# TheNeodev/RVC-MAKER

Hardware: AMD Instinct MI355X
Metric: audio-seconds/sec/GPU (xRT) end-to-end VC, 48k v2; 1/2/4/8 GPU scaling (higher is better)
Workload: dtype f32-equivalent (split-fp16 3-pass MFMA for the generator's convs -- scale from the producer's published |max| -- and ResBlock pairs, split-bf16 6-pass MFMA elsewhere; f32 accumulate; RMVPE f64 with its GRU recurrence f32); 1 GPU; VC.pipeline 48k v2, ContentVec-768, rmvpe f0, one 30 s clip per GPU per step, no index, protect 0.33, clip stream (clip k+1 f0/features under clip k synthesizer); model=RVC v2 48k (NSF-HiFiGAN) + ContentVec + rmvpe, global_batch=1, seq_len=480000, parallelism=utterance-sharded x1

## Files before the change

include/rvc_amd.h:

```cpp
#ifndef RVC_AMD_H
#define RVC_AMD_H

#include <stdint.h>

#ifdef __cplusplus
extern "C" {
#endif

typedef struct ihipStream_t* rvc_stream_t;

enum { RVC_OK = 0, RVC_EINVAL = -22, RVC_EHIP = -5 };

enum {
    RVC_ACT_NONE = 0,
    RVC_ACT_LRELU = 1,
    RVC_ACT_RELU = 2,
    RVC_ACT_TANH = 3,
    RVC_ACT_GELU = 4,
    RVC_ACT_SIGMOID = 5,
    RVC_ACT_LOGCLAMP = 6,
};

const char* rvc_last_error(void);
int rvc_version(void);
// ... 19 lines not shown
    int ntoff, wrap;
    int toff[16];
    const void* wx;
    int wx_nmf, wx_passes;
    const unsigned* amax_in;
    unsigned* amax_out;
    const float* src_x;
    const float* src_w;
    const float* src_b;
    int src_K, src_stride, src_pad, _pad1;
    int64_t src_len, src_bstride;
} rvc_conv1d_args;

int64_t rvc_conv1d_workspace_bytes(const rvc_conv1d_args* a);
int rvc_conv1d_engine(const rvc_conv1d_args* a);
int rvc_conv1d(const rvc_conv1d_args* a, void* ws, int64_t ws_bytes, rvc_stream_t stream);
void rvc_conv1d_set_probe_event(void* hip_event);
int rvc_conv1d_set_stamps(void* buf, int64_t bytes);
int rvc_resblock_set_stamps(void* buf, int64_t bytes);
int rvc_resblock_set_ylds(int on);
int rvc_resblock_set_wide64(int on);
int rvc_conv1d_set_tile_epi(int on);
int rvc_conv1d_set_swz(int on);
int rvc_conv1d_set_f16_fast(int on);
int rvc_conv1d_set_splitk_target(int target);
int rvc_stream_create_cu_mask(const uint32_t* mask, int nwords, rvc_stream_t* out);
int rvc_stream_destroy(rvc_stream_t stream);
int64_t rvc_conv1d_x6_bytes(int64_t nphase, int64_t Ci, int K, int64_t Co);
int rvc_conv1d_pack_x6(const float* w_km, int64_t nphase, int64_t Ci, int K, int64_t Co, void* out, int* nmf_out,
                       rvc_stream_t stream);
// ... 323 lines not shown
```

rvc-maker_amd/csrc/conv1d.hip:

```cpp
#include "rvc_common.h"
#include "x6_common.h"
#include <stdlib.h>
#include <type_traits>
#include <algorithm>

namespace {

constexpr int KCH = 32;
constexpr int NB_MAX = 16;

struct ConvParams {
    const float* x;
    const float* w;
    const float* bias;
    const float* bias2;
    const float* res;
    float* y;
    float* ws;
    int64_t B, Ci, Co, Lin, Lout, ncols;
    int64_t x_bstride, y_bstride, res_bstride, w_bstride;
    int K, stride, dil, pad, groups;
    int nphase, ostride, ooffset;
    int in_act, out_act, accumulate;
    float in_scale, in_slope, out_slope, out_scale;
// ... 51 lines not shown
    else if (t <= -2) yb[m * p.Lout + (-t - 2)] = 0.f;
    return ok ? v : 0.f;
}

template <int ACT, int FM, int FN>
__device__ __forceinline__ void apply_act(floatx4 (&acc)[FM][FN], float slope, float scale) {
#pragma unroll
    for (int i = 0; i < FM; ++i)
#pragma unroll
        for (int j = 0; j < FN; ++j)
#pragma unroll
            for (int r = 0; r < 4; ++r) acc[i][j][r] = act_apply(acc[i][j][r], ACT, slope) * scale;
}

template <int FM, int FN, int WM, int WN>
__device__ __forceinline__ void conv_epilogue(const ConvParams& p, floatx4 (&acc)[FM][FN], int lane, int wm, int wn,
                                              int split, int phase, int b, int g, int Cog, int m0g, int64_t n0) {
    const int ln = lane & 15;
    const int lr = (lane >> 4) * 4;
    if (p.ksplit > 1) {
        float* wsb = p.ws + (((int64_t)split * p.B * p.nphase + (int64_t)b * p.nphase + phase) * p.Co) * p.ncols;
#pragma unroll
        for (int i = 0; i < FM; ++i)
#pragma unroll
            for (int r = 0; r < 4; ++r) {
                const int mg = m0g + wm * 16 * FM + i * 16 + lr + r;
                const int64_t m = (int64_t)g * Cog + mg;
#pragma unroll
                for (int j = 0; j < FN; ++j) {
                    const int64_t n = n0 + wn * 16 * FN + j * 16 + ln;
                    if (mg < Cog && n < p.ncols) wsb[m * p.ncols + n] = acc[i][j][r];
                }
            }
        return;
    }
    int tcol[FN];
#pragma unroll
    for (int j = 0; j < FN; ++j) tcol[j] = out_pos(p, n0 + wn * 16 * FN + j * 16 + ln, phase);
    float* yb = p.y + b * p.y_bstride;
    const float* rb2 = p.res ? p.res + b * p.res_bstride : nullptr;
    const int Lo = (int)p.Lout;
    float amx = 0.f;
#pragma unroll
    for (int i = 0; i < FM; ++i) {
        floatx4 (&av)[1][FN] = *reinterpret_cast<floatx4 (*)[1][FN]>(&acc[i][0]);
        int mrow[4];
        bool mok[4];
#pragma unroll
        for (int r = 0; r < 4; ++r) {
            const int mg = m0g + wm * 16 * FM + i * 16 + lr + r;
            mok[r] = mg < Cog;
            mrow[r] = g * Cog + (mg < Cog ? mg : 0);
            float bs = 0.f;
            if (p.bias) bs = p.bias[mrow[r]];
            if (p.bias2) bs += p.bias2[mrow[r]];
#pragma unroll
            for (int j = 0; j < FN; ++j) av[0][j][r] += bs;
        }
        switch (p.out_act) {
            case RVC_ACT_LRELU: apply_act<RVC_ACT_LRELU, 1, FN>(av, p.out_slope, p.out_scale); break;
            case RVC_ACT_RELU: apply_act<RVC_ACT_RELU, 1, FN>(av, p.out_slope, p.out_scale); break;
            case RVC_ACT_TANH: apply_act<RVC_ACT_TANH, 1, FN>(av, p.out_slope, p.out_scale); break;
            case RVC_ACT_GELU: apply_act<RVC_ACT_GELU, 1, FN>(av, p.out_slope, p.out_scale); break;
            case RVC_ACT_SIGMOID: apply_act<RVC_ACT_SIGMOID, 1, FN>(av, p.out_slope, p.out_scale); break;
            case RVC_ACT_LOGCLAMP: apply_act<RVC_ACT_LOGCLAMP, 1, FN>(av, p.out_slope, p.out_scale); break;
            default: apply_act<RVC_ACT_NONE, 1, FN>(av, p.out_slope, p.out_scale); break;
        }
        if (rb2) {
#pragma unroll
            for (int r = 0; r < 4; ++r)
// ... 11 lines not shown
#pragma unroll
            for (int j = 0; j < FN; ++j) {
                if (mok[r] && tcol[j] >= 0) {
                    yb[mrow[r] * Lo + tcol[j]] = av[0][j][r];
                    amx = fmaxf(amx, fabsf(av[0][j][r]));
                } else if (mok[r] && tcol[j] <= -2) {
                    yb[mrow[r] * Lo + (-tcol[j] - 2)] = 0.f;
                }
            }
    }
    if (p.amax_out) amax_publish(p.amax_out + (int64_t)b * RVC_AMAX_SHARDS, amx);
}

template <int FM, int FN, int WM, int WN>
__device__ __forceinline__ void conv_epilogue_swz(const ConvParams& p, floatx4 (&acc)[FM][FN], int lane, int wm, int wn,
                                                  int phase, int b, int g, int Cog, int m0g, int64_t n0) {
    static_assert(FN % 2 == 0, "column fragments in pairs");
    constexpr int NP = FN / 2;
    const int h = lane >> 5, lc = lane & 31;
    int tcol[NP];
#pragma unroll
    for (int jp = 0; jp < NP; ++jp) tcol[jp] = out_pos(p, n0 + wn * 16 * FN + jp * 32 + lc, phase);
    float* yb = p.y + b * p.y_bstride;
    const float* rb2 = p.res ? p.res + b * p.res_bstride : nullptr;
    const int Lo = (int)p.Lout;
    float amx = 0.f;
#pragma unroll
    for (int i = 0; i < FM; ++i) {
#pragma unroll
        for (int jp = 0; jp < NP; ++jp)
#pragma unroll
            for (int r = 0; r < 4; ++r) {
                const auto sw = __builtin_amdgcn_permlane16_swap(__float_as_uint(acc[i][2 * jp][r]),
                                                                 __float_as_uint(acc[i][2 * jp + 1][r]), false, false);
                acc[i][2 * jp][r] = __uint_as_float(sw[0]);
                acc[i][2 * jp + 1][r] = __uint_as_float(sw[1]);
            }
        floatx4 (&av)[1][FN] = *reinterpret_cast<floatx4 (*)[1][FN]>(&acc[i][0]);
        int mrow[8];
        bool mok[8];
#pragma unroll
        for (int k = 0; k < 8; ++k) {
            const int mg = m0g + wm * 16 * FM + i * 16 + 8 * h + k;
            mok[k] = mg < Cog;
            mrow[k] = g * Cog + (mg < Cog ? mg : 0);
            float bs = 0.f;
            if (p.bias) bs = p.bias[mrow[k]];
            if (p.bias2) bs += p.bias2[mrow[k]];
#pragma unroll
            for (int jp = 0; jp < NP; ++jp) av[0][2 * jp + (k >> 2)][k & 3] += bs;
        }
        switch (p.out_act) {
            case RVC_ACT_LRELU: apply_act<RVC_ACT_LRELU, 1, FN>(av, p.out_slope, p.out_scale); break;
            case RVC_ACT_RELU: apply_act<RVC_ACT_RELU, 1, FN>(av, p.out_slope, p.out_scale); break;
            case RVC_ACT_TANH: apply_act<RVC_ACT_TANH, 1, FN>(av, p.out_slope, p.out_scale); break;
            case RVC_ACT_GELU: apply_act<RVC_ACT_GELU, 1, FN>(av, p.out_slope, p.out_scale); break;
            case RVC_ACT_SIGMOID: apply_act<RVC_ACT_SIGMOID, 1, FN>(av, p.out_slope, p.out_scale); break;
            case RVC_ACT_LOGCLAMP: apply_act<RVC_ACT_LOGCLAMP, 1, FN>(av, p.out_slope, p.out_scale); break;
            default: apply_act<RVC_ACT_NONE, 1, FN>(av, p.out_slope, p.out_scale); break;
        }
        if (rb2) {
#pragma unroll
            for (int k = 0; k < 8; ++k)
// ... 9 lines not shown
                    av[0][2 * jp + (k >> 2)][k & 3] += yb[mrow[k] * Lo + (tcol[jp] >= 0 ? tcol[jp] : 0)];
        }
#pragma unroll
        for (int k = 0; k < 8; ++k)
#pragma unroll
            for (int jp = 0; jp < NP; ++jp) {
                const float v = av[0][2 * jp + (k >> 2)][k & 3];
                if (mok[k] && tcol[jp] >= 0) {
                    yb[mrow[k] * Lo + tcol[jp]] = v;
                    amx = fmaxf(amx, fabsf(v));
                } else if (mok[k] && tcol[jp] <= -2) {
                    yb[mrow[k] * Lo + (-tcol[jp] - 2)] = 0.f;
                }
            }
    }
    if (p.amax_out) amax_publish(p.amax_out + (int64_t)b * RVC_AMAX_SHARDS, amx);
}

template <int FM, int FN, int WM, int WN>
__global__ __launch_bounds__(256) void conv1d_mfma_kernel(ConvParams p) {
    constexpr int BM = 16 * FM * WM;
    constexpr int BN = 16 * FN * WN;
    constexpr int WS = (BM / 32) * 32 + 16 + ((BM % 32) ? 32 : 0);
    constexpr int NA = KCH * BM / 256;
    constexpr bool AVEC_OK = (NA % 4) == 0 && (BM % 4) == 0;
    extern __shared__ __attribute__((aligned(16))) float smem[];
    float* Ws = smem;
    int* koff = (int*)(smem + KCH * WS);
    float* Xs = smem + KCH * WS + KCH;

// ... 285 lines not shown
    if (p.amax_out && !part) amax_publish(p.amax_out + (int64_t)b * RVC_AMAX_SHARDS, amx);
}

template <int FM, int FN, int WM, int WN, int X6_NI, int NP, bool F16, bool SA = false, int LF = 0>
__global__ __launch_bounds__(64 * (WM * WN + 4), (x6_min_blocks<FM, FN, WM * WN, NP>())) void conv_x6_kernel(ConvParams p) {
    static_assert(WM * WN == 4 || WM * WN == 8, "4 or 8 compute waves");
    constexpr int NCW = WM * WN;
    static_assert(NP == 6 || NP == 3 || NP == 1, "6, 3 or 1 passes");
    static_assert(!F16 || NP == 3, "split-fp16: 3 passes");
    static_assert(!SA || (NP == 6 && !F16), "split accumulators: 6-pass split-bf16");
    static_assert(LF == 0 || (F16 && WM * WN == 8), "fast-only loaders: split-fp16 on 8 compute waves");
    constexpr int NPL = NP == 6 ? 3 : (NP == 3 ? 2 : 1);
    constexpr int BM = 16 * FM * WM;
    constexpr int BN = 16 * FN * WN;
    extern __shared__ uint4 xs[];
    const int tid = threadIdx.x, lane = tid & 63, wave = tid >> 6;
    int bx = blockIdx.x, by = blockIdx.y, bz = blockIdx.z;
    if (p.xcd) {
        const int nx = gridDim.x, ny = gridDim.y;
        const int nwg = nx * ny * (int)gridDim.z;
        const int orig = bx + nx * (by + ny * bz);
        const int q = nwg >> 3, r = nwg & 7, xc = orig & 7;
        const int t = (xc < r ? xc * (q + 1) : r * (q + 1) + (xc - r) * q) + (orig >> 3);
        bx = t % nx;
        by = (t / nx) % ny;
        bz = t / (nx * ny);
    }
    int zb = bz;
    const int split = zb % p.ksplit;
    zb /= p.ksplit;
    const int phase = zb % p.nphase;
    const int b = zb / p.nphase;
    const int grp = p.gx6 ? phase : 0;
    const int ophase = p.gx6 ? 0 : phase;
    const int Cog = (int)p.Co;
    const int Cig = (int)p.Ci;
    const int m0g = by * BM;
    const int64_t n0 = (int64_t)bx * BN;
    const int K = p.K, span = p.span;
    const int nch = p.wx_nch, nmf = p.wx_nmf;
    const int ch_beg = split * p.chunks_per_split;
    const int ch_end = min(nch, ch_beg + p.chunks_per_split);
    const int nck = ch_end - ch_beg;
    const int bufsz = NPL * span * 4;
    float* tmax = reinterpret_cast<float*>(xs + 2 * bufsz);
    const int rseed = p.rot ? (bx >> 3) : 0;
    const int rt = rseed % K, rc = (rseed / K) % max(nck, 1);
    auto pchunk = [&](int i) __attribute__((always_inline)) {
        const int c = min(i, nck - 1) + rc;
        return ch_beg + (c >= nck ? c - nck : c);
    };

    if (p.stagger) {
        const int lin = blockIdx.x + gridDim.x * (blockIdx.y + gridDim.y * blockIdx.z);
        if (lin < p.stagger_blocks) {
            const unsigned long long t0 = X6_NOW();
            const unsigned long long d = ((unsigned long long)((lin * 97) & 255) * (unsigned)p.stagger) >> 8;
            while (X6_NOW() - t0 < d) __builtin_amdgcn_s_sleep(2);
        }
    }
// ... 213 lines not shown
                x6_tile_epilogue<BM / 2, BN, 64 * (NCW + 4)>(p, reinterpret_cast<const float*>(xs), tid, split, b, m0g,
                                                             n0);
                __syncthreads();
                __syncthreads();
                x6_tile_epilogue<BM / 2, BN, 64 * (NCW + 4)>(p, reinterpret_cast<const float*>(xs), tid, split, b,
                                                             m0g + BM / 2, n0);
            }
        }
        return;
    }

    const int wm = wave / WN, wn = wave % WN;
    const int s_beg = ch_beg * K, s_end = ch_end * K;
    const uint4* wxp = p.wx + (int64_t)phase * K * nch * nmf * 3 * 64;
    const int mf0 = m0g / 16 + wm * FM;
    auto aload = [&](int i, int tl, uint4 (&a)[NPL][FM]) __attribute__((always_inline)) {
        const int ch = pchunk(i);
        const int t = tl + rt < K ? tl + rt : tl + rt - K;
        const int frag0 = __builtin_amdgcn_readfirstlane((t * nch + ch) * nmf + mf0);
        const uint4* src = wxp + (int64_t)frag0 * 3 * 64;
#pragma unroll
        for (int i = 0; i < FM; ++i)
#pragma unroll
            for (int q = 0; q < NPL; ++q) a[q][i] = src[(i * 3 + q) * 64 + lane];
    };
    floatx4 acc[FM][FN];
    floatx4 acc_lo[SA ? FM : 1][SA ? FN : 1];
#pragma unroll
    for (int i = 0; i < FM; ++i)
#pragma unroll
// ... 53 lines not shown
    uint4 abuf[NB][NPL][FM];
    int li = 0, lt = 0;
#pragma unroll
    for (int i = 0; i < PD; ++i) {
        aload(li, lt, abuf[i]);
        if (++lt == K) { lt = 0; ++li; }
    }
    float tile_rs = 1.f;
    if (wave == 0) X6_STAMP(3, X6_NOW());
    if constexpr (F16) {
        if (!(LF || p.amax_in)) {
            __syncthreads();
            tile_rs = ldexpf(1.f, -f16_exp(fmaxf(fmaxf(tmax[0], tmax[1]), fmaxf(tmax[2], tmax[3]))));
        }
        if (wave == 0) X6_STAMP(4, X6_NOW());
    }
    __syncthreads();
    if constexpr (F16) {
        if (LF || p.amax_in) tile_rs = ldexpf(1.f, -f16_exp(fmaxf(fmaxf(tmax[0], tmax[1]), fmaxf(tmax[2], tmax[3]))));
    }
    if (wave == 0) X6_STAMP(5, X6_NOW());
    const int nsteps = s_end - s_beg;
    int ci = 0, ct = 0;
    for (int s0 = 0; s0 < nsteps; s0 += NB) {
#pragma unroll
        for (int u = 0; u < NB; ++u) {
            aload(li, lt, abuf[(u + PD) % NB]);
            if (++lt == K) { lt = 0; ++li; }
            __builtin_amdgcn_sched_barrier(0);
            if (s0 + u < nsteps) {
// ... 8 lines not shown
    }
    if (wave == 0) X6_STAMP(6, X6_NOW());
    if constexpr (SA) {
#pragma unroll
        for (int i = 0; i < FM; ++i)
#pragma unroll
            for (int j = 0; j < FN; ++j)
#pragma unroll
                for (int r = 0; r < 4; ++r) acc[i][j][r] += acc_lo[i][j][r];
    }
    if (kAblations && (p.dbg & 1)) {
        if (acc[0][0][0] == 1234.5f) p.y[lane] = acc[FM - 1][FN - 1][3];
        return;
    }
    if constexpr (F16) {
        const float* rs = reinterpret_cast<const float*>(p.wx + (int64_t)p.nphase * K * nch * nmf * 3 * 64);
#pragma unroll
        for (int i = 0; i < FM; ++i)
#pragma unroll
            for (int r = 0; r < 4; ++r) {
                const float f = rs[m0g + wm * 16 * FM + i * 16 + lg * 4 + r] * tile_rs;
#pragma unroll
                for (int j = 0; j < FN; ++j) acc[i][j][r] *= f;
            }
    }
    if (BN <= 128 && p.tile_epi) {
        float* ot = reinterpret_cast<float*>(xs);
        constexpr int TS = BN + 4;
#pragma unroll
        for (int i = 0; i < FM; ++i) {
            floatx4 (&av)[1][FN] = *reinterpret_cast<floatx4 (*)[1][FN]>(&acc[i][0]);
            if (p.ksplit == 1) {
#pragma unroll
                for (int r = 0; r < 4; ++r) {
                    const int mg = m0g + wm * 16 * FM + i * 16 + lg * 4 + r;
                    const int mr = mg < Cog ? mg : 0;
                    float bs = 0.f;
                    if (p.bias) bs = p.bias[mr];
                    if (p.bias2) bs += p.bias2[mr];
#pragma unroll
                    for (int j = 0; j < FN; ++j) av[0][j][r] += bs;
                }
                switch (p.out_act) {
                    case RVC_ACT_LRELU: apply_act<RVC_ACT_LRELU, 1, FN>(av, p.out_slope, p.out_scale); break;
                    case RVC_ACT_RELU: apply_act<RVC_ACT_RELU, 1, FN>(av, p.out_slope, p.out_scale); break;
                    case RVC_ACT_TANH: apply_act<RVC_ACT_TANH, 1, FN>(av, p.out_slope, p.out_scale); break;
                    case RVC_ACT_GELU: apply_act<RVC_ACT_GELU, 1, FN>(av, p.out_slope, p.out_scale); break;
                    case RVC_ACT_SIGMOID: apply_act<RVC_ACT_SIGMOID, 1, FN>(av, p.out_slope, p.out_scale); break;
                    case RVC_ACT_LOGCLAMP: apply_act<RVC_ACT_LOGCLAMP, 1, FN>(av, p.out_slope, p.out_scale); break;
                    default: apply_act<RVC_ACT_NONE, 1, FN>(av, p.out_slope, p.out_scale); break;
                }
            }
        }
        auto put = [&](int row0) __attribute__((always_inline)) {
// ... 6 lines not shown
                        ot[(wm * 16 * FM - row0 + i * 16 + lg * 4 + r) * TS + wn * 16 * FN + j * 16 + ln] = acc[i][j][r];
        };
        if (p.tile_epi == 1) {
            put(0);
            __syncthreads();
            x6_tile_epilogue<BM, BN, 64 * (NCW + 4)>(p, ot, tid, split, b, m0g, n0);
        } else if constexpr (WM % 2 == 0) {
            if (wm < WM / 2) put(0);
            __syncthreads();
            x6_tile_epilogue<BM / 2, BN, 64 * (NCW + 4)>(p, ot, tid, split, b, m0g, n0);
            __syncthreads();
            if (wm >= WM / 2) put(BM / 2);
            __syncthreads();
            x6_tile_epilogue<BM / 2, BN, 64 * (NCW + 4)>(p, ot, tid, split, b, m0g + BM / 2, n0);
        }
    } else if (p.swz && p.ksplit == 1) {
        conv_epilogue_swz<FM, FN, WM, WN>(p, acc, lane, wm, wn, ophase, b, grp, Cog, m0g, n0);
    } else {
        conv_epilogue<FM, FN, WM, WN>(p, acc, lane, wm, wn, split, ophase, b, grp, Cog, m0g, n0);
    }
#if RVC_CONV_STAMPS
    if (wave == 0) {
        X6_STAMP(14, X6_NOW());
        __builtin_amdgcn_s_waitcnt(0);
        X6_STAMP(7, X6_NOW());
    }
#endif
}

constexpr int RED_ROWS = 8;
__global__ __launch_bounds__(256) void conv_splitk_reduce(ConvParams p) {
    const int64_t n = (int64_t)blockIdx.x * blockDim.x + threadIdx.x;
    const int bp = blockIdx.z, b = bp / p.nphase;
    const int64_t m0 = (int64_t)blockIdx.y * RED_ROWS;
// ... 298 lines not shown
    }

    if (x6_eligible(a)) {
        cfg.x6 = true;
        static const int w8 = getenv("RVC_X6_W8") ? atoi(getenv("RVC_X6_W8")) : 1;
        const int np = a->wx_passes == 0 || a->wx_passes == RVC_ARITH_FP32_SA ? 6 : a->wx_passes;
        static const int bn256 = getenv("RVC_X6_BN256") ? atoi(getenv("RVC_X6_BN256")) : 1;
        auto round_eff = [](int64_t t) {
            const int64_t n = num_cus();
            return (double)t / (double)(((t + n - 1) / n) * n);
        };
        const int64_t rows128 = (Cog + 127) / 128, nb = a->B * a->nphase;
        const bool fills256 = round_eff(rows128 * ((ncols + 255) / 256) * nb) >=
                              round_eff(rows128 * ((ncols + 127) / 128) * nb) - 0.05;
        if (Cog > 64 && w8 && bn256 && a->stride == 1 && 255 + max_tap_off(a) + 1 <= 64 * X6_NI_MAX - 2 &&
            (bn256 == 2 || np == RVC_ARITH_F16X3) && (fills256 || bn256 == 3))
            cfg = {2, 8, 4, 2, true};
        else if (Cog > 64 && w8) cfg = {2, 4, 4, 2, true};
        else if (Cog > 64) cfg = {4, 4, 2, 2, true};
        else if (Cog > 32 && w8 && np >= 3) cfg = {2, 2, 2, 4, true};
        else if (Cog > 32) cfg = {2, 4, 2, 2, true};
        else if (Cog > 16) cfg = {2, 2, 1, 4, true};
        else cfg = {1, 2, 1, 4, true};
        RVC_CHECK_ARG(a->wx_passes != RVC_ARITH_FP32_SA || x6_sa_tile(cfg.FM, cfg.FN, cfg.WM, cfg.WN),
                      "conv1d: RVC_ARITH_FP32_SA has no split-accumulator kernel for the %dx%d tile on %d waves "
                      "(engine switches changed?)", 16 * cfg.FM * cfg.WM, 16 * cfg.FN * cfg.WN, cfg.WM * cfg.WN);
        const int BM = 16 * cfg.FM * cfg.WM, BN = 16 * cfg.FN * cfg.WN;
        p.span = (BN - 1) * a->stride + max_tap_off(a) + 1;
        p.span_s = p.span;
        p.rows_max = 0;
// ... 10 lines not shown
            p.nphase = a->groups;
            p.Ci = Cig;
            p.Co = Cog;
            p.chunks_per_split = p.wx_nch;
            p.ksplit = 1;
        }
        lds = (size_t)2 * (p.wx_passes == 6 || p.wx_passes == RVC_ARITH_FP32_SA ? 3 : (p.wx_passes == 1 ? 1 : 2)) *
              p.span * 64 + 16;
        static const int tepi_env = getenv("RVC_X6_TILE_EPI") ? atoi(getenv("RVC_X6_TILE_EPI")) : 0;
        const int tepi = g_tile_epi >= 0 ? g_tile_epi : tepi_env;
        const size_t tile_bytes = (size_t)BM * (BN + 4) * 4;
        const bool plain = a->nphase == 1 && a->ostride == 1 && a->ooffset == 0 && !a->wrap && !(p.dbg & 1) &&
                           BN <= 128;
        p.tile_epi = !(tepi && plain && a->groups == 1) ? 0
                     : tile_bytes <= lds ? 1 : (cfg.WM % 2 == 0 && tile_bytes / 2 <= lds) ? 2 : 0;
        grid = dim3(cdiv(ncols, BN), (unsigned)p.mtiles_per_group, (unsigned)(a->B * p.nphase * p.ksplit));
        RVC_CHECK_ARG(grid.y < 65536 && grid.z < 65536, "conv1d: grid too large");
        static const int stagger = getenv("RVC_X6_STAGGER") ? atoi(getenv("RVC_X6_STAGGER")) : 0;
        static const int stagger_rounds = getenv("RVC_X6_STAGGER_ROUNDS") ? atoi(getenv("RVC_X6_STAGGER_ROUNDS")) : 2;
        const int64_t nblk = (int64_t)grid.x * grid.y * grid.z;
        if (stagger > 0 && nblk >= stagger_rounds * (int64_t)num_cus()) {
            p.stagger = stagger;
            p.stagger_blocks = num_cus();
        }
        return RVC_OK;
    }

    if (Cog % 48 == 0 && Cog % 64 != 0) cfg = {3, 1, 1, 4, false};
    else if (Cog <= 16) cfg = {1, 4, 1, 4, false};
    else if (Cog <= 32) cfg = {2, 4, 1, 4, false};
// ... 146 lines not shown
    hipLaunchKernelGGL(rowscale_fin_kernel, dim3(cdiv(nmf * 16, 256)), dim3(256), 0, s, rs, nmf * 16);
    hipLaunchKernelGGL(pack_f16_kernel, dim3(cdiv(total, 256)), dim3(256), 0, s, w_km, total, (int)Ci, K, (int)Co, nch,
                       nmf, (const float*)rs, (uint4*)out);
    RVC_HIP(hipGetLastError());
    *nmf_out = nmf;
    return RVC_OK;
}

extern "C" int rvc_conv1d_engine(const rvc_conv1d_args* a) {
    ConvParams p;
    Cfg cfg;
    dim3 grid;
    size_t lds;
    if (plan(a, p, cfg, grid, lds) != RVC_OK) return -1;
    return cfg.x6 ? 1 : 0;
}

extern "C" int64_t rvc_conv1d_workspace_bytes(const rvc_conv1d_args* a) {
    ConvParams p;
    Cfg cfg;
    dim3 grid;
    size_t lds;
    if (plan(a, p, cfg, grid, lds) != RVC_OK) return -1;
    if (p.ksplit <= 1) return 0;
    return (int64_t)p.ksplit * p.B * p.nphase * p.Co * p.ncols * 4;
}

extern "C" int rvc_conv1d_set_splitk_target(int target) {
    const int prev = g_splitk_target;
    g_splitk_target = target < 0 ? -1 : target;
// ... 98 lines not shown
```

rvc-maker_amd/rvc_amd/_lib.py:

```python
from __future__ import annotations

import ctypes
import os
from ctypes import POINTER, c_double, c_float, c_int, c_int64, c_uint64, c_void_p

LIB_PATH = os.environ.get("RVC_AMD_LIB") or os.path.join(
    os.path.dirname(os.path.dirname(os.path.abspath(__file__))), "lib", "librvc_amd.so")

ACT_NONE, ACT_LRELU, ACT_RELU, ACT_TANH, ACT_GELU, ACT_SIGMOID, ACT_LOGCLAMP = 0, 1, 2, 3, 4, 5, 6


class Conv1dArgs(ctypes.Structure):
    _fields_ = [("x", c_void_p), ("w", c_void_p), ("bias", c_void_p), ("bias2", c_void_p), ("res", c_void_p),
                ("y", c_void_p),
                ("B", c_int64), ("Ci", c_int64), ("Co", c_int64), ("Lin", c_int64), ("Lout", c_int64),
                ("ncols", c_int64), ("x_bstride", c_int64), ("y_bstride", c_int64), ("res_bstride", c_int64),
                ("w_bstride", c_int64),
                ("K", c_int), ("stride", c_int), ("dil", c_int), ("pad", c_int), ("groups", c_int),
                ("nphase", c_int), ("ostride", c_int), ("ooffset", c_int),
                ("in_act", c_int), ("out_act", c_int), ("accumulate", c_int), ("_pad0", c_int),
                ("in_scale", c_float), ("in_slope", c_float), ("out_slope", c_float), ("out_scale", c_float),
                ("ntoff", c_int), ("wrap", c_int), ("toff", c_int * 16),
                ("wx", c_void_p), ("wx_nmf", c_int), ("wx_passes", c_int),
                ("amax_in", c_void_p), ("amax_out", c_void_p),
# ... 86 lines not shown
    "rvc_conv1d": [POINTER(Conv1dArgs), c_void_p, c_int64, c_void_p],
    "rvc_conv1d_workspace_bytes": [POINTER(Conv1dArgs)],
    "rvc_conv1d_set_probe_event": [c_void_p],
    "rvc_conv1d_set_stamps": [c_void_p, c_int64],
    "rvc_resblock_set_stamps": [c_void_p, c_int64],
    "rvc_resblock_set_ylds": [c_int],
    "rvc_resblock_set_wide64": [c_int],
    "rvc_conv1d_set_tile_epi": [c_int],
    "rvc_conv1d_set_swz": [c_int],
    "rvc_conv1d_set_f16_fast": [c_int],
    "rvc_bigru64_set_f32": [c_int],
    "rvc_conv1d_set_splitk_target": [c_int],
    "rvc_stream_create_cu_mask": [c_void_p, c_int, POINTER(c_void_p)],
    "rvc_stream_destroy": [c_void_p],
    "rvc_conv1d_engine": [POINTER(Conv1dArgs)],
    "rvc_conv1d_x6_bytes": [c_int64, c_int64, c_int, c_int64],
    "rvc_conv1d_pack_x6": [c_void_p, c_int64, c_int64, c_int, c_int64, c_void_p, POINTER(c_int), c_void_p],
    "rvc_conv1d_f16_bytes": [c_int64, c_int64, c_int, c_int64],
    "rvc_pm_frames": [c_int64],
    "rvc_pm_work_bytes": [c_int64],
    "rvc_pm_f0": [c_void_p, c_int64, c_void_p, c_void_p, c_void_p, c_int64, c_void_p, c_void_p],
    "rvc_pm_post": [c_void_p, c_int64, c_int64, ctypes.c_double, c_void_p, c_void_p, c_void_p, c_void_p],
    "rvc_conv1d_pack_f16": [c_void_p, c_int64, c_int64, c_int, c_int64, c_void_p, POINTER(c_int), c_void_p],
    "rvc_attention_workspace_bytes": [POINTER(AttnArgs)],
    "rvc_attention": [POINTER(AttnArgs), c_void_p, c_int64, c_void_p],
    "rvc_attention_amax": [POINTER(AttnArgs), c_void_p, c_void_p, c_int64, c_void_p],
    "rvc_attention_ex": [POINTER(AttnArgs), c_void_p, c_void_p, c_void_p, c_int64, c_void_p],
    "rvc_attention_set_f16": [c_int],
    "rvc_layernorm_cf_amax": [c_void_p, c_void_p, c_void_p, c_void_p, c_void_p, c_int64, c_int64, c_int64, c_float,
                              c_void_p, c_void_p],
# ... 154 lines not shown
```

rvc-maker_amd/rvc_amd/ops.py:

```python
from __future__ import annotations

import ctypes
import math
import os

import torch

from . import _lib
from ._lib import ACT_GELU, ACT_LOGCLAMP, ACT_LRELU, ACT_NONE, ACT_RELU, ACT_SIGMOID, ACT_TANH, check


def _stream():
    return ctypes.c_void_p(torch.cuda.current_stream().cuda_stream)


def _p(t):
    if t is None:
        return None
    if not t.is_cuda or t.dtype not in (torch.float32, torch.int64, torch.int32):
        raise TypeError(f"rvc_amd: expected a CUDA f32/int tensor, got {t.dtype} on {t.device}")
    return ctypes.c_void_p(t.data_ptr())


def pack_km(w: torch.Tensor, groups: int = 1) -> torch.Tensor:
# ... 156 lines not shown
    def __getitem__(self, k):
        w = self.B * AMAX_SHARDS
        return self.words[k * w:(k + 1) * w]


def amax_value(cell, b=0):
    import numpy as np
    words = cell[b * AMAX_SHARDS:(b + 1) * AMAX_SHARDS].cpu().numpy().astype(np.int32)
    return float(words.view(np.float32).max())


LAST_CONV_FLOPS = 0.0
LAST_CONV_ENGINE = 0
LAST_CONV_PASSES = 0
LAST_CONV_WS = 0
_WS = {}
_WS_PRIVATE = None


class private_workspaces:

    def __init__(self, store: dict):
        self.store = store

    def __enter__(self):
        global _WS_PRIVATE
        self.prev, _WS_PRIVATE = _WS_PRIVATE, self.store
        return self.store

    def __exit__(self, *a):
        global _WS_PRIVATE
        _WS_PRIVATE = self.prev
# ... 14 lines not shown
def _room(t):
    return t.untyped_storage().nbytes() // t.element_size() - t.storage_offset()


def _shape3(x):
    if x.dim() == 2:
        return 1, x.shape[0], x.shape[1]
    return x.shape[0], x.shape[1], x.shape[2]


def conv1d(x, w, Ci, Co, K, *, bias=None, bias2=None, stride=1, pad=0, dil=1, groups=1, Lout=None, ncols=0,
           nphase=1, ostride=1, ooffset=0, out=None, res=None, in_act=ACT_NONE, in_slope=0.0, in_scale=1.0,
           out_act=ACT_NONE, out_slope=0.0, out_scale=1.0, accumulate=False, B=None, Lin=None, x_bstride=0,
           w_bstride=0, y_bstride=0, res_bstride=0, toff=None, wrap=0, flops=None, wx=None, wx_nmf=0,
           amax_in=None, amax_out=None, src=None):
    global LAST_CONV_FLOPS, LAST_CONV_ENGINE, LAST_CONV_PASSES, LAST_CONV_WS
    if B is None:
        B, Cx, Lx = _shape3(x)
        if Lin is None:
            Lin = Lx
        if Cx != Ci:
            raise ValueError(f"conv1d: x has {Cx} channels, weight expects {Ci}")
        if not x.is_contiguous():
            raise ValueError("conv1d: x must be contiguous")
    if Lout is None:
        Lout = (Lin + 2 * pad - dil * (K - 1) - 1) // stride + 1
    if Lout <= 0:
        raise ValueError("conv1d: empty output")
    Cig = Ci // groups
    need_w = nphase * Cig * K * Co
    if w.numel() < need_w or (w_bstride and w.numel() < need_w + (B - 1) * w_bstride):
# ... 41 lines not shown
    if wx is not None:
        passes = conv_passes(K, Ci // groups, stride, toff is not None, amax_in is not None)
        a.wx, a.wx_nmf, a.wx_passes = ctypes.c_void_p(wx.data_ptr(passes)), wx_nmf, passes
    if flops is None:
        valid = (Lout // wrap - 2) * (wrap - 2) if wrap else (ncols or Lout) * nphase
        flops = 2.0 * B * Co * Cig * K * min(valid, Lout)
    LAST_CONV_FLOPS = flops
    lib = _lib.load()
    need = lib.rvc_conv1d_workspace_bytes(ctypes.byref(a))
    if need < 0:
        raise RuntimeError(f"rvc_amd: conv1d plan failed: {lib.rvc_last_error().decode()}")
    ws = _workspace(out.device, need) if need else None
    LAST_CONV_WS = need
    LAST_CONV_ENGINE = lib.rvc_conv1d_engine(ctypes.byref(a))
    LAST_CONV_PASSES = a.wx_passes if LAST_CONV_ENGINE == 1 else 0
    check(lib.rvc_conv1d(ctypes.byref(a), _p(ws), need, _stream()), "conv1d")
    return out


FUSED_RB = os.environ.get("RVC_AMD_FUSED_RB", "1") != "0"
RB_PASSES = (6, 3, 1, F16X3)


RB_F16_KMIN = int(os.environ.get("RVC_AMD_RB_F16_KMIN", "3"))


def rb_passes(K):
    if _PRECISION == "fp32" and F16_MIX and K >= RB_F16_KMIN:
        return F16X3
    return PASSES[_PRECISION]
# ... 615 lines not shown
```

Baseline: 1141 audio-s/s.

## Stage per-row scale and bias in LDS and add row-wise x6 conv epilogue

Loads each tile's per-row f16 rescale and bias values once into a small LDS table before the main barrier, so the epilogues read from LDS and no longer issue repeated global bias/scale loads. For the 256-wide (FN=8) tiles it adds a new row-oriented epilogue that precomputes 32-bit column offsets, specializes on residual/accumulate/all-in-bounds cases, and applies transcendental activations through a per-wave LDS scratch (reusing the X buffers) to limit register pressure. The wide tile config is also restricted to Cog%16==0 and lengths under 2^26 so the 32-bit offsets stay valid. A tile-query API is added for diagnostics. The cost is extra LDS per block and more code paths to keep consistent.

```diff
diff --git a/include/rvc_amd.h b/include/rvc_amd.h
--- a/include/rvc_amd.h
+++ b/include/rvc_amd.h
@@ -57,6 +57,7 @@
 
 int64_t rvc_conv1d_workspace_bytes(const rvc_conv1d_args* a);
 int rvc_conv1d_engine(const rvc_conv1d_args* a);
+int rvc_conv1d_tile(const rvc_conv1d_args* a);
 int rvc_conv1d(const rvc_conv1d_args* a, void* ws, int64_t ws_bytes, rvc_stream_t stream);
 void rvc_conv1d_set_probe_event(void* hip_event);
 int rvc_conv1d_set_stamps(void* buf, int64_t bytes);
diff --git a/rvc-maker_amd/csrc/conv1d.hip b/rvc-maker_amd/csrc/conv1d.hip
--- a/rvc-maker_amd/csrc/conv1d.hip
+++ b/rvc-maker_amd/csrc/conv1d.hip
@@ -89,24 +89,46 @@
 }
 
 template <int FM, int FN, int WM, int WN>
+__device__ __forceinline__ void conv_store_partial(const ConvParams& p, floatx4 (&acc)[FM][FN], int lane, int wm, int wn,
+                                                   int split, int phase, int b, int g, int Cog, int m0g, int64_t n0) {
+    const int ln = lane & 15;
+    const int lr = (lane >> 4) * 4;
+    float* wsb = p.ws + (((int64_t)split * p.B * p.nphase + (int64_t)b * p.nphase + phase) * p.Co) * p.ncols;
+#pragma unroll
+    for (int i = 0; i < FM; ++i)
+#pragma unroll
+        for (int r = 0; r < 4; ++r) {
+            const int mg = m0g + wm * 16 * FM + i * 16 + lr + r;
+            const int64_t m = (int64_t)g * Cog + mg;
+#pragma unroll
+            for (int j = 0; j < FN; ++j) {
+                const int64_t n = n0 + wn * 16 * FN + j * 16 + ln;
+                if (mg < Cog && n < p.ncols) wsb[m * p.ncols + n] = acc[i][j][r];
+            }
+        }
+}
+
+template <bool TB, int BM>
+__device__ __forceinline__ float epi_bias(const ConvParams& p, const float* tb, int rl, int mrow) {
+    float bs = 0.f;
+    if constexpr (TB) {
+        bs = tb[BM + rl];
+        bs += tb[2 * BM + rl];
+    } else {
+        if (p.bias) bs = p.bias[mrow];
+        if (p.bias2) bs += p.bias2[mrow];
+    }
+    return bs;
+}
+
+template <int FM, int FN, int WM, int WN, bool TB = false>
 __device__ __forceinline__ void conv_epilogue(const ConvParams& p, floatx4 (&acc)[FM][FN], int lane, int wm, int wn,
-                                              int split, int phase, int b, int g, int Cog, int m0g, int64_t n0) {
+                                              int split, int phase, int b, int g, int Cog, int m0g, int64_t n0,
+                                              const float* tb = nullptr) {
     const int ln = lane & 15;
     const int lr = (lane >> 4) * 4;
     if (p.ksplit > 1) {
-        float* wsb = p.ws + (((int64_t)split * p.B * p.nphase + (int64_t)b * p.nphase + phase) * p.Co) * p.ncols;
-#pragma unroll
-        for (int i = 0; i < FM; ++i)
-#pragma unroll
-            for (int r = 0; r < 4; ++r) {
-                const int mg = m0g + wm * 16 * FM + i * 16 + lr + r;
-                const int64_t m = (int64_t)g * Cog + mg;
-#pragma unroll
-                for (int j = 0; j < FN; ++j) {
-                    const int64_t n = n0 + wn * 16 * FN + j * 16 + ln;
-                    if (mg < Cog && n < p.ncols) wsb[m * p.ncols + n] = acc[i][j][r];
-                }
-            }
+        conv_store_partial<FM, FN, WM, WN>(p, acc, lane, wm, wn, split, phase, b, g, Cog, m0g, n0);
         return;
     }
     int tcol[FN];
@@ -126,9 +148,7 @@
             const int mg = m0g + wm * 16 * FM + i * 16 + lr + r;
             mok[r] = mg < Cog;
             mrow[r] = g * Cog + (mg < Cog ? mg : 0);
-            float bs = 0.f;
-            if (p.bias) bs = p.bias[mrow[r]];
-            if (p.bias2) bs += p.bias2[mrow[r]];
+            const float bs = epi_bias<TB, 16 * FM * WM>(p, tb, wm * 16 * FM + i * 16 + lr + r, mrow[r]);
 #pragma unroll
             for (int j = 0; j < FN; ++j) av[0][j][r] += bs;
         }
@@ -170,7 +190,8 @@
 
 template <int FM, int FN, int WM, int WN>
 __device__ __forceinline__ void conv_epilogue_swz(const ConvParams& p, floatx4 (&acc)[FM][FN], int lane, int wm, int wn,
-                                                  int phase, int b, int g, int Cog, int m0g, int64_t n0) {
+                                                  int phase, int b, int g, int Cog, int m0g, int64_t n0,
+                                                  const float* tb) {
     static_assert(FN % 2 == 0, "column fragments in pairs");
     constexpr int NP = FN / 2;
     const int h = lane >> 5, lc = lane & 31;
@@ -200,9 +221,7 @@
             const int mg = m0g + wm * 16 * FM + i * 16 + 8 * h + k;
             mok[k] = mg < Cog;
             mrow[k] = g * Cog + (mg < Cog ? mg : 0);
-            float bs = 0.f;
-            if (p.bias) bs = p.bias[mrow[k]];
-            if (p.bias2) bs += p.bias2[mrow[k]];
+            const float bs = epi_bias<true, 16 * FM * WM>(p, tb, wm * 16 * FM + i * 16 + 8 * h + k, mrow[k]);
 #pragma unroll
             for (int jp = 0; jp < NP; ++jp) av[0][2 * jp + (k >> 2)][k & 3] += bs;
         }
@@ -242,6 +261,166 @@
                 }
             }
     }
+    if (p.amax_out) amax_publish(p.amax_out + (int64_t)b * RVC_AMAX_SHARDS, amx);
+}
+
+template <int FM, int FN, int WM, int WN, bool SWZ, bool PART = false>
+__device__ __forceinline__ void conv_epilogue_rows(const ConvParams& p, floatx4 (&acc)[FM][FN], int lane, int wm, int wn,
+                                                   int split, int phase, int b, int g, int Cog, int m0g, int64_t n0,
+                                                   const float* tb, float* scr) {
+    static_assert(!(SWZ && PART), "split-K partial tiles keep the accumulator layout");
+    static_assert(FN % 2 == 0, "column fragments in pairs");
+    constexpr int BM = 16 * FM * WM;
+    constexpr int NV = SWZ ? FN / 2 : FN;
+    constexpr int NR = SWZ ? 8 : 4;
+    constexpr int CW = SWZ ? 32 : 16;
+#define X6_EL(kr, jv) acc[i][SWZ ? 2 * (jv) + ((kr) >> 2) : (jv)][SWZ ? ((kr) & 3) : (kr)]
+    const int lrow = SWZ ? (lane >> 5) * 8 : (lane >> 4) * 4;
+    const int lcol = lane & (CW - 1);
+    const int Lo = PART ? (int)p.ncols : (int)p.Lout;
+    const int64_t c0 = n0 + wn * 16 * FN + lcol;
+    auto col_pos = [&](int jv) __attribute__((always_inline)) {
+        const int64_t n = c0 + jv * CW;
+        if constexpr (PART) return n < p.ncols ? (int)n : -1;
+        else return out_pos(p, n, phase);
+    };
+    uint32_t voff[NV];
+    unsigned okm = 0;
+#pragma unroll
+    for (int jv = 0; jv < NV; ++jv) {
+        const int t = col_pos(jv);
+        okm |= (unsigned)(t >= 0) << jv;
+        voff[jv] = (uint32_t)(lrow * Lo + (t >= 0 ? t : 0)) * 4u;
+    }
+    float* yb = PART ? p.ws + (((int64_t)split * p.B * p.nphase + (int64_t)b * p.nphase + phase) * p.Co) * p.ncols
+                     : p.y + b * p.y_bstride;
+    const float* rb2 = !PART && p.res ? p.res + b * p.res_bstride : nullptr;
+    const bool accum = !PART && p.accumulate;
+    const bool allok = __builtin_amdgcn_ballot_w64(okm != (1u << NV) - 1u) == 0;
+    const size_t rowb = (size_t)Lo * 4;
+    float amx = 0.f;
+    auto run = [&](auto spec_c) __attribute__((always_inline)) {
+        constexpr int SPEC = decltype(spec_c)::value;
+        const bool all = SPEC < 0 ? allok : true;
+        const bool has_res = SPEC < 0 ? rb2 != nullptr : (SPEC & 1) != 0;
+        const bool has_acc = SPEC < 0 ? accum : (SPEC & 2) != 0;
+#pragma unroll
+        for (int i = 0; i < FM; ++i) {
+            const int srow = m0g + wm * 16 * FM + i * 16;
+            if (srow >= Cog) continue;
+            if constexpr (SWZ) {
+#pragma unroll
+                for (int jp = 0; jp < FN / 2; ++jp)
+#pragma unroll
+                    for (int r = 0; r < 4; ++r) {
+                        const auto sw = __builtin_amdgcn_permlane16_swap(__float_as_uint(acc[i][2 * jp][r]),
+                                                                         __float_as_uint(acc[i][2 * jp + 1][r]), false, false);
+                        acc[i][2 * jp][r] = __uint_as_float(sw[0]);
+                        acc[i][2 * jp + 1][r] = __uint_as_float(sw[1]);
+                    }
+            }
+            if constexpr (!PART) {
+                floatx4 (&av)[1][FN] = *reinterpret_cast<floatx4 (*)[1][FN]>(&acc[i][0]);
+#pragma unroll
+                for (int kr = 0; kr < NR; ++kr) {
+                    const float bs = epi_bias<true, BM>(p, tb, wm * 16 * FM + i * 16 + lrow + kr, 0);
+#pragma unroll
+                    for (int jv = 0; jv < NV; ++jv) X6_EL(kr, jv) += bs;
+                }
+                const int oa = p.out_act;
+                if (oa == RVC_ACT_TANH || oa == RVC_ACT_GELU || oa == RVC_ACT_SIGMOID || oa == RVC_ACT_LOGCLAMP) {
+#pragma unroll
+                    for (int q0 = 0; q0 < FN; q0 += 4) {
+#pragma unroll
+                        for (int q = 0; q < 4; ++q)
+#pragma unroll
+                            for (int r = 0; r < 4; ++r) scr[(q * 4 + r) * 64 + lane] = av[0][q0 + q][r];
+#pragma unroll 1
+                        for (int e = 0; e < 16; ++e) {
+                            const float v = scr[e * 64 + lane];
+                            scr[e * 64 + lane] = act_apply(v, oa, p.out_slope) * p.out_scale;
+                        }
+#pragma unroll
+                        for (int q = 0; q < 4; ++q)
+#pragma unroll
+                            for (int r = 0; r < 4; ++r) av[0][q0 + q][r] = scr[(q * 4 + r) * 64 + lane];
+                    }
+                } else if (oa == RVC_ACT_LRELU) {
+                    apply_act<RVC_ACT_LRELU, 1, FN>(av, p.out_slope, p.out_scale);
+                } else if (oa == RVC_ACT_RELU) {
+                    apply_act<RVC_ACT_RELU, 1, FN>(av, p.out_slope, p.out_scale);
+                } else {
+                    apply_act<RVC_ACT_NONE, 1, FN>(av, p.out_slope, p.out_scale);
+                }
+            }
+            const int64_t ro = (int64_t)(g * Cog + srow) * Lo;
+            char* ybase = reinterpret_cast<char*>(yb + ro);
+            if (has_res) {
+                const char* rbase = reinterpret_cast<const char*>(rb2 + ro);
+                float rv[NR][NV];
+#pragma unroll
+                for (int kr = 0; kr < NR; ++kr)
+#pragma unroll
+                    for (int jv = 0; jv < NV; ++jv) rv[kr][jv] = *reinterpret_cast<const float*>(rbase + kr * rowb + voff[jv]);
+#pragma unroll
+                for (int kr = 0; kr < NR; ++kr)
+#pragma unroll
+                    for (int jv = 0; jv < NV; ++jv) X6_EL(kr, jv) += rv[kr][jv];
+            }
+            if (has_acc) {
+                float yv[NR][NV];
+#pragma unroll
+                for (int kr = 0; kr < NR; ++kr)
+#pragma unroll
+                    for (int jv = 0; jv < NV; ++jv) yv[kr][jv] = *reinterpret_cast<const float*>(ybase + kr * rowb + voff[jv]);
+#pragma unroll
+                for (int kr = 0; kr < NR; ++kr)
+#pragma unroll
+                    for (int jv = 0; jv < NV; ++jv) X6_EL(kr, jv) += yv[kr][jv];
+            }
+            if (all) {
+#pragma unroll
+                for (int kr = 0; kr < NR; ++kr)
+#pragma unroll
+                    for (int jv = 0; jv < NV; ++jv) {
+                        const float v = X6_EL(kr, jv);
+                        *reinterpret_cast<float*>(ybase + kr * rowb + voff[jv]) = v;
+                        amx = fmaxf(amx, fabsf(v));
+                    }
+            } else {
+#pragma unroll
+                for (int kr = 0; kr < NR; ++kr)
+#pragma unroll
+                    for (int jv = 0; jv < NV; ++jv) {
+                        const float v = X6_EL(kr, jv);
+                        if ((okm >> jv) & 1u) {
+                            *reinterpret_cast<float*>(ybase + kr * rowb + voff[jv]) = v;
+                            amx = fmaxf(amx, fabsf(v));
+                        }
+                    }
+            }
+        }
+    };
+    if (!allok) run(std::integral_constant<int, -1>{});
+    else if (rb2 && accum) run(std::integral_constant<int, 3>{});
+    else if (rb2) run(std::integral_constant<int, 1>{});
+    else if (accum) run(std::integral_constant<int, 2>{});
+    else run(std::integral_constant<int, 0>{});
+    if constexpr (PART) return;
+    if (p.wrap) {
+#pragma unroll 1
+        for (int i = 0; i < FM; ++i) {
+            const int srow = m0g + wm * 16 * FM + i * 16;
+            if (srow >= Cog) continue;
+#pragma unroll 1
+            for (int jv = 0; jv < NV; ++jv) {
+                const int t = col_pos(jv);
+                if (t > -2) continue;
+                for (int kr = 0; kr < NR; ++kr) yb[(int64_t)(g * Cog + srow + lrow + kr) * Lo + (-t - 2)] = 0.f;
+            }
+        }
+    }
+#undef X6_EL
     if (p.amax_out) amax_publish(p.amax_out + (int64_t)b * RVC_AMAX_SHARDS, amx);
 }
 
@@ -557,7 +736,8 @@
     constexpr int BM = 16 * FM * WM;
     constexpr int BN = 16 * FN * WN;
     extern __shared__ uint4 xs[];
-    const int tid = threadIdx.x, lane = tid & 63, wave = tid >> 6;
+    const int tid = threadIdx.x, lane = tid & 63;
+    const int wave = __builtin_amdgcn_readfirstlane(tid >> 6);
     int bx = blockIdx.x, by = blockIdx.y, bz = blockIdx.z;
     if (p.xcd) {
         const int nx = gridDim.x, ny = gridDim.y;
@@ -587,6 +767,7 @@
     const int nck = ch_end - ch_beg;
     const int bufsz = NPL * span * 4;
     float* tmax = reinterpret_cast<float*>(xs + 2 * bufsz);
+    float* etab = tmax + 4;
     const int rseed = p.rot ? (bx >> 3) : 0;
     const int rt = rseed % K, rc = (rseed / K) % max(nck, 1);
     auto pchunk = [&](int i) __attribute__((always_inline)) {
@@ -830,6 +1011,17 @@
     const int s_beg = ch_beg * K, s_end = ch_end * K;
     const uint4* wxp = p.wx + (int64_t)phase * K * nch * nmf * 3 * 64;
     const int mf0 = m0g / 16 + wm * FM;
+    const float* rscale = reinterpret_cast<const float*>(p.wx + (int64_t)p.nphase * K * nch * nmf * 3 * 64);
+    float et_rs = 1.f, et_b1 = 0.f, et_b2 = -0.f;
+    if (tid < BM) {
+        const int mg = m0g + tid;
+        const int mr = grp * Cog + (mg < Cog ? mg : 0);
+        const float* wz = reinterpret_cast<const float*>(p.wx);
+        if constexpr (F16) et_rs = rscale[mg];
+        const float v1 = *(p.bias ? p.bias + mr : wz), v2 = *(p.bias2 ? p.bias2 + mr : wz);
+        et_b1 = p.bias ? v1 : 0.f;
+        et_b2 = p.bias2 ? v2 : -0.f;
+    }
     auto aload = [&](int i, int tl, uint4 (&a)[NPL][FM]) __attribute__((always_inline)) {
         const int ch = pchunk(i);
         const int t = tl + rt < K ? tl + rt : tl + rt - K;
@@ -913,6 +1105,11 @@
             tile_rs = ldexpf(1.f, -f16_exp(fmaxf(fmaxf(tmax[0], tmax[1]), fmaxf(tmax[2], tmax[3]))));
         }
         if (wave == 0) X6_STAMP(4, X6_NOW());
+    }
+    if (tid < BM) {
+        etab[tid] = et_rs;
+        etab[BM + tid] = et_b1;
+        etab[2 * BM + tid] = et_b2;
     }
     __syncthreads();
     if constexpr (F16) {
@@ -951,12 +1148,11 @@
         return;
     }
     if constexpr (F16) {
-        const float* rs = reinterpret_cast<const float*>(p.wx + (int64_t)p.nphase * K * nch * nmf * 3 * 64);
 #pragma unroll
         for (int i = 0; i < FM; ++i)
 #pragma unroll
             for (int r = 0; r < 4; ++r) {
-                const float f = rs[m0g + wm * 16 * FM + i * 16 + lg * 4 + r] * tile_rs;
+                const float f = etab[wm * 16 * FM + i * 16 + lg * 4 + r] * tile_rs;
 #pragma unroll
                 for (int j = 0; j < FN; ++j) acc[i][j][r] *= f;
             }
@@ -971,10 +1167,7 @@
 #pragma unroll
                 for (int r = 0; r < 4; ++r) {
                     const int mg = m0g + wm * 16 * FM + i * 16 + lg * 4 + r;
-                    const int mr = mg < Cog ? mg : 0;
-                    float bs = 0.f;
-                    if (p.bias) bs = p.bias[mr];
-                    if (p.bias2) bs += p.bias2[mr];
+                    const float bs = epi_bias<true, BM>(p, etab, wm * 16 * FM + i * 16 + lg * 4 + r, 0);
 #pragma unroll
                     for (int j = 0; j < FN; ++j) av[0][j][r] += bs;
                 }
@@ -1011,10 +1204,20 @@
             __syncthreads();
             x6_tile_epilogue<BM / 2, BN, 64 * (NCW + 4)>(p, ot, tid, split, b, m0g + BM / 2, n0);
         }
+    } else if constexpr (FN == 8) {
+        static_assert(NCW * 16 * 64 * 4 <= 2 * 256 * 64, "the rolled activations need 4 KB per compute wave of the X "
+                                                         "buffers' smallest size (2 buffers x 1 plane x span 256 x 64 B)");
+        static_assert(!X6_NOBAR || RVC_CONV_ABLATIONS, "the X buffers are reused after the last chunk's barrier");
+        float* scr = reinterpret_cast<float*>(xs) + wave * (16 * 64);
+        if (p.ksplit > 1)
+            conv_epilogue_rows<FM, FN, WM, WN, false, true>(p, acc, lane, wm, wn, split, ophase, b, grp, Cog, m0g, n0, etab, scr);
+        else if (p.swz)
+            conv_epilogue_rows<FM, FN, WM, WN, true>(p, acc, lane, wm, wn, 0, ophase, b, grp, Cog, m0g, n0, etab, scr);
+        else conv_epilogue_rows<FM, FN, WM, WN, false>(p, acc, lane, wm, wn, 0, ophase, b, grp, Cog, m0g, n0, etab, scr);
     } else if (p.swz && p.ksplit == 1) {
-        conv_epilogue_swz<FM, FN, WM, WN>(p, acc, lane, wm, wn, ophase, b, grp, Cog, m0g, n0);
+        conv_epilogue_swz<FM, FN, WM, WN>(p, acc, lane, wm, wn, ophase, b, grp, Cog, m0g, n0, etab);
     } else {
-        conv_epilogue<FM, FN, WM, WN>(p, acc, lane, wm, wn, split, ophase, b, grp, Cog, m0g, n0);
+        conv_epilogue<FM, FN, WM, WN, true>(p, acc, lane, wm, wn, split, ophase, b, grp, Cog, m0g, n0, etab);
     }
 #if RVC_CONV_STAMPS
     if (wave == 0) {
@@ -1343,6 +1546,7 @@
         const bool fills256 = round_eff(rows128 * ((ncols + 255) / 256) * nb) >=
                               round_eff(rows128 * ((ncols + 127) / 128) * nb) - 0.05;
         if (Cog > 64 && w8 && bn256 && a->stride == 1 && 255 + max_tap_off(a) + 1 <= 64 * X6_NI_MAX - 2 &&
+            Cog % 16 == 0 && a->Lout < (1ll << 26) && ncols < (1ll << 26) &&
             (bn256 == 2 || np == RVC_ARITH_F16X3) && (fills256 || bn256 == 3))
             cfg = {2, 8, 4, 2, true};
         else if (Cog > 64 && w8) cfg = {2, 4, 4, 2, true};
@@ -1383,6 +1587,7 @@
                            BN <= 128;
         p.tile_epi = !(tepi && plain && a->groups == 1) ? 0
                      : tile_bytes <= lds ? 1 : (cfg.WM % 2 == 0 && tile_bytes / 2 <= lds) ? 2 : 0;
+        lds += (size_t)3 * BM * 4;
         grid = dim3(cdiv(ncols, BN), (unsigned)p.mtiles_per_group, (unsigned)(a->B * p.nphase * p.ksplit));
         RVC_CHECK_ARG(grid.y < 65536 && grid.z < 65536, "conv1d: grid too large");
         static const int stagger = getenv("RVC_X6_STAGGER") ? atoi(getenv("RVC_X6_STAGGER")) : 0;
@@ -1559,6 +1764,15 @@
     size_t lds;
     if (plan(a, p, cfg, grid, lds) != RVC_OK) return -1;
     return cfg.x6 ? 1 : 0;
+}
+
+extern "C" int rvc_conv1d_tile(const rvc_conv1d_args* a) {
+    ConvParams p;
+    Cfg cfg;
+    dim3 grid;
+    size_t lds;
+    if (plan(a, p, cfg, grid, lds) != RVC_OK) return -1;
+    return (16 * cfg.FM * cfg.WM) << 16 | (16 * cfg.FN * cfg.WN);
 }
 
 extern "C" int64_t rvc_conv1d_workspace_bytes(const rvc_conv1d_args* a) {
diff --git a/rvc-maker_amd/rvc_amd/_lib.py b/rvc-maker_amd/rvc_amd/_lib.py
--- a/rvc-maker_amd/rvc_amd/_lib.py
+++ b/rvc-maker_amd/rvc_amd/_lib.py
@@ -124,6 +124,7 @@
     "rvc_stream_create_cu_mask": [c_void_p, c_int, POINTER(c_void_p)],
     "rvc_stream_destroy": [c_void_p],
     "rvc_conv1d_engine": [POINTER(Conv1dArgs)],
+    "rvc_conv1d_tile": [POINTER(Conv1dArgs)],
     "rvc_conv1d_x6_bytes": [c_int64, c_int64, c_int, c_int64],
     "rvc_conv1d_pack_x6": [c_void_p, c_int64, c_int64, c_int, c_int64, c_void_p, POINTER(c_int), c_void_p],
     "rvc_conv1d_f16_bytes": [c_int64, c_int64, c_int, c_int64],
diff --git a/rvc-maker_amd/rvc_amd/ops.py b/rvc-maker_amd/rvc_amd/ops.py
--- a/rvc-maker_amd/rvc_amd/ops.py
+++ b/rvc-maker_amd/rvc_amd/ops.py
@@ -194,8 +194,15 @@
 LAST_CONV_ENGINE = 0
 LAST_CONV_PASSES = 0
 LAST_CONV_WS = 0
+_LAST_CONV_ARGS = None
 _WS = {}
 _WS_PRIVATE = None
+
+
+def last_conv_tile():
+    if _LAST_CONV_ARGS is None:
+        return 0, 0
+    return divmod(_lib.load().rvc_conv1d_tile(ctypes.byref(_LAST_CONV_ARGS)), 1 << 16)
 
 
 class private_workspaces:
@@ -240,7 +247,7 @@
            out_act=ACT_NONE, out_slope=0.0, out_scale=1.0, accumulate=False, B=None, Lin=None, x_bstride=0,
            w_bstride=0, y_bstride=0, res_bstride=0, toff=None, wrap=0, flops=None, wx=None, wx_nmf=0,
            amax_in=None, amax_out=None, src=None):
-    global LAST_CONV_FLOPS, LAST_CONV_ENGINE, LAST_CONV_PASSES, LAST_CONV_WS
+    global LAST_CONV_FLOPS, LAST_CONV_ENGINE, LAST_CONV_PASSES, LAST_CONV_WS, _LAST_CONV_ARGS
     if B is None:
         B, Cx, Lx = _shape3(x)
         if Lin is None:
@@ -312,6 +319,7 @@
     LAST_CONV_WS = need
     LAST_CONV_ENGINE = lib.rvc_conv1d_engine(ctypes.byref(a))
     LAST_CONV_PASSES = a.wx_passes if LAST_CONV_ENGINE == 1 else 0
+    _LAST_CONV_ARGS = a
     check(lib.rvc_conv1d(ctypes.byref(a), _p(ws), need, _stream()), "conv1d")
     return out
 
```

After: 1195 audio-s/s, median of 6. 1.05x the previous value.
